# JialeTao/MRFA

Hardware: AMD Instinct MI355X
Metric: frames/sec (256x256 source+driving pair) fwd+bwd (higher is better)
Workload: dtype f32; 1 GPU; vox1.yaml MTIA (TokenPose_B) prior + DenseMotion + RaftFlow refinement, 256x256, bs=8/GPU, fwd+bwd+clip+Adam, train-mode BN, surrogate L1 loss; global_batch=8, parallelism=dp1, prior=mtia, background_predictor=False, sync_bn=False, launch=hipGraph, optimizer=FlatAdam (K20), mfma=bf16x6

## Files before the change

mrfa_amd/build.py:

```python
import glob
import os
import subprocess
import sys

HERE = os.path.dirname(os.path.abspath(__file__))
ROOT = os.path.dirname(HERE)
CSRC = os.path.join(HERE, "csrc")
LIBDIR = os.path.join(HERE, "_lib")
LIB = os.path.join(LIBDIR, "libmrfa_hip.so")
SOURCES = ["error.cpp", "conv_plan.hip", "conv_mfma.hip", "conv_split.hip", "conv_halo.hip", "conv_small.hip", "conv_lean.hip", "wgrad_mfma.hip", "wgrad_split.hip", "wgrad_halo.hip", "wgrad_small.hip", "wgrad_lean.hip", "conv_fewout.hip", "conv_fewout3.hip", "layout.hip", "pack_multi.hip", "norm.hip", "sample.hip", "elementwise.hip", "optim.hip", "tokenpose.hip", "attention_mfma.hip", "losses.hip", "prior.hip", "pose.hip", "metrics.hip", "frames.hip"]
FLAGS = ["--offload-arch=gfx950", "-O3", "-std=c++17", "-fPIC", "-I" + os.path.join(ROOT, "include"), "-I" + CSRC,
         "-Wno-unused-result"]
CSRC_DATA = os.path.join(HERE, "csrc_data")
DATA_LIB = os.path.join(LIBDIR, "libmrfa_data_hip.so")
DATA_FLAGS = FLAGS + ["-I" + CSRC_DATA, "-ffp-contract=off", "-fhip-fp32-correctly-rounded-divide-sqrt"]


def _stale(out, deps):
    if not os.path.exists(out):
        return True
    t = os.path.getmtime(out)
    return any(os.path.getmtime(d) > t for d in deps)


def data_sources() -> list:
    return ["error.cpp"] + sorted(os.path.basename(p) for p in glob.glob(os.path.join(CSRC_DATA, "*.hip")))


def build(force: bool = False, verbose: bool = True) -> str:
    os.makedirs(LIBDIR, exist_ok=True)
    hipcc = os.environ.get("HIPCC", "/opt/rocm/bin/hipcc")
    headers = [os.path.join(ROOT, "include", "mrfa_hip.h")] + sorted(glob.glob(os.path.join(CSRC, "*.h")))
    data_headers = headers + [os.path.join(ROOT, "include", h) for h in ("mrfa_data_hip.h", "mrfa_resize_hip.h")] \
        + sorted(glob.glob(os.path.join(CSRC_DATA, "*.h")))
    units = [(CSRC, src, "", FLAGS, headers) for src in SOURCES] + [(CSRC_DATA, src, "data_", DATA_FLAGS, data_headers) for src in data_sources()]
    objs = {LIB: [], DATA_LIB: []}
    procs = []
    for srcdir, src, prefix, flags, deps in units:
        sp = os.path.join(srcdir, src)
        if not os.path.exists(sp):
            raise FileNotFoundError(sp)
        obj = os.path.join(LIBDIR, prefix + os.path.splitext(src)[0] + ".o")
        objs[DATA_LIB if prefix else LIB].append(obj)
        if force or _stale(obj, [sp] + deps):
            cmd = [hipcc] + flags + (["-x", "hip"] if src.endswith(".cpp") else []) + ["-c", sp, "-o", obj]
            if verbose:
                print("[mrfa_amd.build]", " ".join(cmd), flush=True)
            procs.append((src, subprocess.Popen(cmd)))
    for src, pr in procs:
        if pr.wait() != 0:
            raise RuntimeError(f"hipcc failed on {src}")
    for out, os_ in objs.items():
        if force or _stale(out, os_):
            cmd = [hipcc, "--offload-arch=gfx950", "-shared", "-fPIC", "-o", out] + os_
            if verbose:
                print("[mrfa_amd.build]", " ".join(cmd), flush=True)
            subprocess.check_call(cmd)
    return LIB


if __name__ == "__main__":
    build(force="--force" in sys.argv)
    print(LIB)
    print(DATA_LIB)
```

mrfa_amd/csrc/common.h:

```cpp
#pragma once
#include <hip/hip_runtime.h>
#include <stdio.h>
#include <string.h>
#include "mrfa_hip.h"

typedef float f32x16 __attribute__((ext_vector_type(16)));
typedef float f32x4 __attribute__((ext_vector_type(4)));

void mrfa_set_error(const char* fmt, ...);

struct MrfaTuning {
    int conv_small;
    int conv_halo, conv_halo_min_tiles, conv_halo_pr, conv_halo_phase, conv_halo_bn256, conv_halo_bn192, conv_halo_bn64_fill;
    int conv_lean, conv_lean_min_wgs, conv_lean_geo, gemm_lean;
    int wgrad_halo, wgrad_halo_min_wgs, wgrad_halo_target_wgs, wgrad_halo_phase, wgrad_lean;
    int conv_fewout3, attention_mfma;
};
extern MrfaTuning g_tune;

struct HaloGeo { int PR, BN; bool phase; };

enum class ConvFamily { lean, gemm_lean, small, halo, halo_dgrad, rows_split, rows_f32, refused };
struct ConvPlan {
    ConvFamily family;
    char error[256];
    long long M;
    int KT;
    int lean_geo, gemm_cfg, small_tm, small_tn;
    HaloGeo halo;
    int BM, BN, splitk;
    bool w8;
    bool fused;
    bool fin_in_launch;
    bool reads_w;
    int last_config;
    bool groups_ok, bst_ok, stride2_ok, mask_ok, phase_dgrad_ok;
};
ConvPlan plan_conv(const mrfa_conv_params& p);

enum class WgradFamily { lean, small, halo, tiled, refused };
struct WgradPlan {
    WgradFamily family;
    char error[192];
    long long M;
    bool lean, small;
    bool groups_ok, stride2_ok;
};
WgradPlan plan_wgrad(const mrfa_wgrad_params& p);

int mrfa_conv_split_launch(hipStream_t st, const mrfa_conv_params& p, int KT, long long M, int splitk, int BN);
bool mrfa_conv_halo_eligible(const mrfa_conv_params& p, HaloGeo* geo);
int mrfa_conv_halo_launch(hipStream_t st, const mrfa_conv_params& p, const HaloGeo& geo);
int mrfa_wgrad_split_launch(hipStream_t st, const mrfa_wgrad_params& p, dim3 grid, long long M, long long kps, int tiles_n, int nsplit, int inner,
                            int total_splits, int taps, long long partial_stride, int BM, int BN);

bool mrfa_wgrad_halo_eligible(const mrfa_wgrad_params& p);
int mrfa_wgrad_halo_launch(hipStream_t st, const mrfa_wgrad_params& p);

bool mrfa_fewout3_wgrad(hipStream_t st, const float* x, int ldx, int N, int H, int W, int Cin, const float* dy, int lddy, int Cout, int R, int pad,
                        float* dw, float* dbias, int* rc);

int mrfa_conv_lean_pick(const mrfa_conv_params& p);
int mrfa_conv_lean_launch(hipStream_t st, const mrfa_conv_params& p, int geo);
int mrfa_gemm_lean_pick(const mrfa_conv_params& p, long long M);
int mrfa_gemm_lean_launch(hipStream_t st, const mrfa_conv_params& p, long long M, int cfg);

bool mrfa_conv_small_eligible(const mrfa_conv_params& p, long long M);
int mrfa_conv_small_launch(hipStream_t st, const mrfa_conv_params& p, long long M, int tm, int tn);

bool mrfa_attention_mfma_ok(int d, int n, const void* qkv, int ld, const void* out, int ldo, const void* dout, int lddo, const void* dqkv, int lddq);
int mrfa_attention_fwd_mfma(hipStream_t st, const float* qkv, int ld, int B, int n, int heads, int d, float scale, float* out, int ldo, float* lse);
int mrfa_attention_bwd_mfma(hipStream_t st, const float* qkv, int ld, const float* out, int ldo, const float* dout, int lddo, const float* lse,
                            float* delta, int B, int n, int heads, int d, float scale, float* dqkv, int lddq);

bool mrfa_wgrad_lean_eligible(const mrfa_wgrad_params& p);
int mrfa_wgrad_lean_multi(hipStream_t st, const mrfa_wgrad_params* ps, int n, unsigned char* taken);

bool mrfa_wgrad_small_eligible(const mrfa_wgrad_params& p, long long M);
int mrfa_wgrad_small_launch(hipStream_t st, const mrfa_wgrad_params& p, long long M);

#define MRFA_CHECK_ARG(cond, ...)                      \
    do {                                               \
        if (!(cond)) {                                 \
            mrfa_set_error(__VA_ARGS__);               \
            return 1;                                  \
        }                                              \
    } while (0)

#define MRFA_CHECK_LAUNCH(name)                                                   \
    do {                                                                          \
        hipError_t e_ = hipGetLastError();                                        \
        if (e_ != hipSuccess) {                                                   \
            mrfa_set_error("%s: launch failed: %s", name, hipGetErrorString(e_)); \
            return 2;                                                             \
        }                                                                         \
    } while (0)

static inline bool aligned16(const void* p) { return (reinterpret_cast<uintptr_t>(p) & 15u) == 0; }
static inline int cdiv(long long a, long long b) { return (int)((a + b - 1) / b); }

static inline int stream_grid(long long work_items, int block) {
    long long g = (work_items + block - 1) / block;
    if (g < 1) g = 1;
    if (g > 256 * 16) g = 256 * 16;
    return (int)g;
}

__device__ __forceinline__ int xcd_tile_index() {
    const int per_xcd = (int)gridDim.x >> 3;
    return (int)(blockIdx.x & 7) * per_xcd + (int)(blockIdx.x >> 3);
}

__device__ __forceinline__ void chain_prio() {
    __builtin_amdgcn_s_setprio(3);
}

__device__ __forceinline__ int stat_group(const mrfa_conv_params& p, long long row, long long M) {
    return p.groups > 1 ? (int)(row / (M / p.groups)) : 0;
}
__device__ __forceinline__ double* stat_slot(const mrfa_conv_params& p, int group, unsigned slot) {
    return p.stats + ((size_t)group * MRFA_STATS_SLOTS + slot % MRFA_STATS_SLOTS) * 2 * p.Cout;
}
static inline long long group_rows(const mrfa_conv_params& p, long long M) {
    if (p.groups <= 1) return M;
    return (p.N % p.groups) == 0 ? M / p.groups : 0;
}

__device__ __forceinline__ bool splitk_last_arriver(unsigned* ticket, unsigned nsplit) {
    __shared__ unsigned s_sk_ticket;
    asm volatile("s_waitcnt vmcnt(0)" ::: "memory");
    __syncthreads();
    if (threadIdx.x == 0) s_sk_ticket = __hip_atomic_fetch_add(ticket, 1u, __ATOMIC_RELAXED, __HIP_MEMORY_SCOPE_AGENT);
    __syncthreads();
    return s_sk_ticket == nsplit - 1;
}

__device__ __forceinline__ bool fin_last_arriver(unsigned* counter, unsigned participants, int idx) {
    __shared__ unsigned s_fin_ticket;
    asm volatile("s_waitcnt vmcnt(0)" ::: "memory");
    __syncthreads();
    if (threadIdx.x == 0) {
        if (idx < 0) {
            s_fin_ticket = __hip_atomic_fetch_add(counter, 1u, __ATOMIC_RELAXED, __HIP_MEMORY_SCOPE_AGENT) == participants - 1;
        } else {
            const unsigned nsh = participants < 8u ? participants : 8u, sh = (unsigned)idx % nsh;
            const unsigned mine = participants / nsh + (sh < participants % nsh ? 1u : 0u);
            unsigned last = 0;
            if (__hip_atomic_fetch_add(counter + 1 + sh, 1u, __ATOMIC_RELAXED, __HIP_MEMORY_SCOPE_AGENT) == mine - 1)
                last = __hip_atomic_fetch_add(counter, 1u, __ATOMIC_RELAXED, __HIP_MEMORY_SCOPE_AGENT) == nsh - 1;
            s_fin_ticket = last;
        }
    }
    __syncthreads();
    return s_fin_ticket != 0;
}

__device__ __forceinline__ double fin_slot_sum(const double* first, size_t stride) {
    double v[MRFA_STATS_SLOTS];
#pragma unroll
    for (int s = 0; s < MRFA_STATS_SLOTS; ++s) v[s] = __hip_atomic_load(first + (size_t)s * stride, __ATOMIC_RELAXED, __HIP_MEMORY_SCOPE_AGENT);
    double t = 0.0;
#pragma unroll
    for (int s = 0; s < MRFA_STATS_SLOTS; ++s) t += v[s];
    return t;
}

__device__ __forceinline__ void fused_bn_finalize(const mrfa_conv_params& p, unsigned participants, int idx = -1, double* scratch = nullptr, int scratch_n = 0) {
    if (!fin_last_arriver(p.fin_counter, participants, idx)) return;
    const double cnt = (double)p.fin_count;
    const int G = p.groups > 1 ? p.groups : 1;
    const int C2 = 2 * p.Cout;
    const bool par = scratch != nullptr && scratch_n >= G * C2;
    if (par) {
        for (int o = threadIdx.x; o < G * C2; o += blockDim.x) scratch[o] = fin_slot_sum(p.stats + (size_t)(o / C2) * MRFA_STATS_SLOTS * C2 + o % C2, (size_t)C2);
        __syncthreads();
    }
    for (int c = threadIdx.x; c < p.Cout; c += blockDim.x) {
        float rm = p.fin_rmean ? p.fin_rmean[c] : 0.f, rv = p.fin_rmean ? p.fin_rvar[c] : 0.f;
        for (int g = 0; g < G; ++g) {
            const double* sg = p.stats + (size_t)g * MRFA_STATS_SLOTS * C2;
            const double t1 = par ? scratch[g * C2 + c] : fin_slot_sum(sg + c, (size_t)C2);
            const double t2 = par ? scratch[g * C2 + p.Cout + c] : fin_slot_sum(sg + p.Cout + c, (size_t)C2);
            const double m = t1 / cnt;
            double var = t2 / cnt - m * m;
            if (var < 0.0) var = 0.0;
            const float mean = (float)m, invstd = (float)(1.0 / sqrt(var + (double)p.fin_eps));
            const double unb = p.fin_count > 1 ? var * cnt / (cnt - 1.0) : var;
            rm = (1.f - p.fin_momentum) * rm + p.fin_momentum * mean;
            rv = (1.f - p.fin_momentum) * rv + p.fin_momentum * (float)unb;
            const float sc = p.fin_gamma[c] * invstd;
            const int gc = g * p.Cout + c;
            p.fin_scale[gc] = sc;
            p.fin_shift[gc] = p.fin_beta[c] - mean * sc;
            if (p.fin_mean) p.fin_mean[gc] = mean;
            if (p.fin_invstd) p.fin_invstd[gc] = invstd;
        }
        if (p.fin_rmean) { p.fin_rmean[c] = rm; p.fin_rvar[c] = rv; }
    }
}

__device__ __forceinline__ float wave_sum(float v) {
#pragma unroll
    for (int o = 32; o > 0; o >>= 1) v += __shfl_xor(v, o, 64);
    return v;
}
```

mrfa_amd/csrc/conv_plan.hip:

```cpp
#include "common.h"
#include <stdarg.h>

MrfaTuning g_tune = {
     1,
     1,  128,  0,  1,  1,
     1,  1,
     1,  128,  -1,
     1,
     1,  192,  256,  1,
     1,
     1,  1,
};

enum TuneKind { T_ON, T_INT, T_NONNEG, T_NONNEG_ON, T_LEVEL, T_POS };
static const struct { const char* key; int* field; TuneKind kind; } TUNING_KEYS[] = {
    {"conv_small", &g_tune.conv_small, T_ON},
    {"conv_halo", &g_tune.conv_halo, T_ON},
    {"conv_halo_min_tiles", &g_tune.conv_halo_min_tiles, T_INT},
    {"conv_halo_pr", &g_tune.conv_halo_pr, T_INT},
    {"conv_halo_phase", &g_tune.conv_halo_phase, T_ON},
    {"conv_halo_bn256", &g_tune.conv_halo_bn256, T_ON},
    {"conv_halo_bn192", &g_tune.conv_halo_bn192, T_ON},
    {"conv_halo_bn64_fill", &g_tune.conv_halo_bn64_fill, T_ON},
    {"conv_lean", &g_tune.conv_lean, T_ON},
    {"conv_lean_min_wgs", &g_tune.conv_lean_min_wgs, T_NONNEG},
    {"conv_lean_geo", &g_tune.conv_lean_geo, T_INT},
    {"gemm_lean", &g_tune.gemm_lean, T_LEVEL},
    {"wgrad_halo", &g_tune.wgrad_halo, T_ON},
    {"wgrad_halo_min_wgs", &g_tune.wgrad_halo_min_wgs, T_NONNEG},
    {"wgrad_halo_target_wgs", &g_tune.wgrad_halo_target_wgs, T_POS},
    {"wgrad_halo_phase", &g_tune.wgrad_halo_phase, T_NONNEG_ON},
    {"wgrad_lean", &g_tune.wgrad_lean, T_ON},
    {"conv_fewout3", &g_tune.conv_fewout3, T_ON},
    {"attention_mfma", &g_tune.attention_mfma, T_ON},
};

extern "C" int mrfa_set_tuning(const char* key, int value) {
    if (!key) return -1;
    for (const auto& k : TUNING_KEYS) {
        if (strcmp(key, k.key)) continue;
        const int prev = *k.field;
        switch (k.kind) {
            case T_ON: *k.field = value != 0; break;
            case T_INT: *k.field = value; break;
            case T_NONNEG: if (value >= 0) *k.field = value; break;
            case T_NONNEG_ON: if (value >= 0) *k.field = value != 0; break;
            case T_LEVEL: if (value >= 0) *k.field = value > 2 ? 2 : value; break;
            case T_POS: if (value > 0) *k.field = value; break;
        }
        return prev;
    }
    return -1;
}

namespace {
constexpr int BK = 32;

template <typename Plan>
Plan& refuse(Plan& c, const char* fmt, ...) {
    va_list ap;
    va_start(ap, fmt);
    vsnprintf(c.error, sizeof(c.error), fmt, ap);
    va_end(ap);
    c.family = decltype(c.family)::refused;
    return c;
}

void plan_rows(ConvPlan& c, const mrfa_conv_params& p, int mode) {
    const bool flat = p.kflat > 0;
    const long long M = c.M;
    const int KT = c.KT;
    const int nb = p.nbatch > 1 ? p.nbatch : 1;
    int BN = 128;
    {
        const int cands[4] = {128, 96, 64, 32};
        const double pen[4] = {1.0, 1.08, 1.16, 1.3};
        double best = 1e18;
        for (int i = 0; i < 4; ++i) {
            if (cands[i] == 96 && flat) continue;
            const double cost = (double)cdiv(p.Cout, cands[i]) * cands[i] * pen[i];
            if (cost < best) { best = cost; BN = cands[i]; }
        }
    }
    if (mode >= 1 && !flat && p.Cout >= 32) BN = p.Cout <= 64 ? 64 : 128;
    auto ntiles = [&](int bm, int bn) { return ((M + bm - 1) / bm) * cdiv(p.Cout, bn) * nb; };
    int BM = 128;
    if (BN == 96 && ntiles(128, 96) < 384) BN = 128;
    if (BN == 128) { if (M <= 32) BM = 32; else if (M <= 64) BM = 64; }
    else if (BN == 64 && M <= 64) BM = 64;
    int splitk = 1;
    const bool auto_split = (p.splitk == 0);
    if (p.splitk > 1) splitk = p.splitk;
    {
        const bool short_k_big_m = KT < 32 && M > 4096;
        const bool grouped_stats = p.groups > 1 && p.stats && !(p.sk_ticket && !p.accumulate);
        const int max_split = (auto_split && !short_k_big_m && !grouped_stats) ? (KT / 2 > 0 ? KT / 2 : 1) : 1;
        long long t = ntiles(BM, BN);
        if (t < 384 && !(short_k_big_m && t >= 128)) {
            const bool half_target = auto_split && p.sk_ticket && !p.accumulate && KT >= 72 && KT <= 320 && BM == 128 && t >= 8 && t <= 16;
            int want = (int)(((half_target ? 256 : 512) + t - 1) / t);
            if (auto_split) splitk = want <= max_split ? want : max_split;
            const int min_bm = (BN == 128) ? 32 : (BN == 64 ? 64 : 128);
            while (!half_target && ntiles(BM, BN) * splitk < 384 && BM > min_bm) {
                BM >>= 1;
                if (auto_split) {
                    t = ntiles(BM, BN);
                    want = (int)((512 + t - 1) / t);
                    splitk = want <= max_split ? want : max_split;
                }
            }
            if (splitk < 1) splitk = 1;
        }
    }
    bool w8 = false;
    if (p.tile) {
        BM = p.tile >> 16; BN = p.tile & 0x7fff; w8 = (p.tile & 0x8000) != 0;
        if (p.splitk >= 1) splitk = p.splitk;
    } else if (BM == 128 && BN == 128 && !flat) {
        w8 = true;
    }
    const bool split_operand = mode >= 1 && BM == 128 && (BN == 128 || BN == 64) && !flat;
    c.family = split_operand ? ConvFamily::rows_split : ConvFamily::rows_f32;
    c.BM = BM;
    c.BN = BN;
    c.w8 = w8;
    c.splitk = splitk;
    c.fused = splitk > 1 && p.sk_ticket && !p.accumulate;
    c.fin_in_launch = p.fin_scale && nb == 1 && (splitk == 1 || c.fused);
    c.reads_w = !(split_operand && mode != 3 && p.w_split);
    c.last_config = (BM << 16) | (BN << 4) | ((flat ? 1 : 0) << 1) | (splitk > 1 ? 1 : 0) | (split_operand ? 4 : 0);
}
}

ConvPlan plan_conv(const mrfa_conv_params& p) {
    ConvPlan c = {};
    const int mode = mrfa_get_mfma_mode();
    const bool flat = p.kflat > 0;
    c.M = (long long)p.N * p.Hout * p.Wout;
    c.KT = ((flat ? p.kflat : p.R * p.S * p.Cin) + BK - 1) / BK;
    c.splitk = 1;
    c.reads_w = true;
    c.fin_in_launch = p.fin_scale != nullptr;

    c.lean_geo = flat ? -1 : mrfa_conv_lean_pick(p);
    c.gemm_cfg = (flat || c.lean_geo >= 0) ? -1 : mrfa_gemm_lean_pick(p, c.M);
    const bool lean = c.lean_geo >= 0, gemm = c.gemm_cfg >= 0;
    const bool small = !lean && !gemm && g_tune.conv_small && mrfa_conv_small_eligible(p, c.M);
    const bool halo = !flat && mrfa_conv_halo_eligible(p, &c.halo);

    const long long rows = group_rows(p, c.M);
    c.groups_ok = p.groups <= 1 || !(p.stats || p.fin_scale || p.bst_x || p.in_scale) ||
                  (p.nbatch <= 1 && p.splitk <= 1 && rows > 0 &&
                   (lean || gemm || (!p.in_scale && ((rows % 128) == 0 || small || (p.stride <= 1 && halo)))));
    c.bst_ok = p.stats && !p.fin_scale && p.stride >= 0 && !flat && (lean || gemm || small);
    c.stride2_ok = p.stride == 2 && p.Hout == (p.Hin + 2 * p.pad - p.R) / 2 + 1 && p.Wout == (p.Win + 2 * p.pad - p.S) / 2 + 1 &&
                   (flat ? (!p.ups && p.nbatch <= 1 && p.splitk <= 1 && p.ktab) : small);
    c.mask_ok = halo;
    c.phase_dgrad_ok = p.ups == 2 && halo;

    if (!(p.x && p.w)) return refuse(c, "conv2d: null pointer");
    if (!(p.N > 0 && p.Cin > 0 && p.Cout > 0 && p.Hout > 0 && p.Wout > 0)) return refuse(c, "conv2d: bad sizes");
    if (!(p.R >= 1 && p.S >= 1 && p.R <= 15 && p.S <= 15)) return refuse(c, "conv2d: kernel size %dx%d unsupported", p.R, p.S);
    if (!((p.w_ld % 4) == 0 && aligned16(p.w))) return refuse(c, "conv2d: packed weight must be 16-B aligned, w_ld %% 4 == 0");
    if (!flat && (p.Cin % 32) != 0) return refuse(c, "conv2d: chunked mode needs Cin %% 32 == 0 (got %d); use flat mode", p.Cin);
    if (!flat && !((p.ldx % 4) == 0 && aligned16(p.x))) return refuse(c, "conv2d: chunked mode needs 16-B aligned x and ldx %% 4 == 0");
    if (!flat && p.in_scale && !(aligned16(p.in_scale) && aligned16(p.in_shift))) return refuse(c, "conv2d: in_scale/in_shift alignment");
    if (flat && !(p.ktab != nullptr && aligned16(p.ktab))) return refuse(c, "conv2d: flat mode needs a 16-B aligned ktab");
    if (lean) {
        c.family = ConvFamily::lean;
        c.reads_w = false;
        c.last_config = (32 << 16) | (32 << 4) | 4 | (1 << 27);
        return c;
    }
    if (gemm) {
        c.family = ConvFamily::gemm_lean;
        c.reads_w = false;
        c.last_config = (64 << 16) | (64 << 4) | 4 | (1 << 26);
        return c;
    }
    if (small) {
        c.family = ConvFamily::small;
        const int ncols = (p.Cout + 15) / 16 * 16;
        auto waves = [&](int wm, int wn) { return ((c.M + wm - 1) / wm) * ((ncols + wn - 1) / wn); };
        int tm = 2, tn = 2;
        if (waves(32, 32) < 2048) { tm = 1; tn = 2; }
        if (tm == 1 && waves(16, 32) < 2048) { tn = 1; }
        if (ncols % 32 != 0 && tn == 2 && ncols < 32) tn = 1;
        if (p.groups > 1 && tm == 2 && (rows % 128) != 0) tm = 1;
        c.small_tm = tm;
        c.small_tn = tn;
        c.last_config = (16 << 16) | (16 << 4) | 8;
        return c;
    }
    if (p.stride < 0 || p.stride > 2 || (p.stride == 2 && !(flat && !p.ups && p.nbatch <= 1)))
        return refuse(c, "conv2d: stride = %d is only implemented by the one-wave-per-tile kernel and by flat-K launches: ask mrfa_conv2d_stride_supported() first", p.stride);
    if (p.mask && !halo) return refuse(c, "conv2d: `mask` is only honoured by the patch-tiled kernel: ask mrfa_conv2d_mask_supported() first");
    if (p.ups == 2 && !halo)
        return refuse(c, "conv2d: ups = 2 (phase data gradient of a fused-upsample layer) is only implemented for the shapes mrfa_conv2d_phase_dgrad_supported() reports");
    if (halo) {
        c.family = p.ups == 2 ? ConvFamily::halo_dgrad : ConvFamily::halo;
        c.reads_w = false;
        c.last_config = (128 << 16) | ((p.Cout <= 64 ? 64 : 128) << 4) | 4 | (1 << 28);
        return c;
    }
    plan_rows(c, p, mode);
    return c;
}

WgradPlan plan_wgrad(const mrfa_wgrad_params& p) {
    WgradPlan c = {};
    const bool flat = p.kflat > 0;
    c.M = (long long)p.N * p.Hout * p.Wout;
    c.lean = mrfa_wgrad_lean_eligible(p);
    c.small = g_tune.conv_small && mrfa_wgrad_small_eligible(p, c.M);
    c.groups_ok = p.groups <= 1 || !p.in_scale || c.lean;
    c.stride2_ok = p.stride == 2 && p.Hout == (p.Hin + 2 * p.pad - p.R) / 2 + 1 && p.Wout == (p.Win + 2 * p.pad - p.S) / 2 + 1 && c.small;
    if (!(p.x && p.dy && p.dw)) return refuse(c, "wgrad: null pointer");
    if (!flat && !((p.ldx % 4) == 0 && aligned16(p.x))) return refuse(c, "wgrad: x must be a 16-B aligned view with ld %% 4 == 0");
    if (flat && !p.ktab) return refuse(c, "wgrad: flat mode needs ktab");
    if (!(c.M < (1ll << 31) - 64)) return refuse(c, "wgrad: too many pixels");
    if (p.in_scale && c.lean) { c.family = WgradFamily::lean; return c; }
    if (!c.groups_ok) return refuse(c, "wgrad: groups = %d with a prologue is only implemented where mrfa_conv2d_wgrad_groups_supported() says so", p.groups);
    if (c.small) { c.family = WgradFamily::small; return c; }
    if (p.stride > 1) return refuse(c, "wgrad: stride = %d is only implemented by the small-problem kernel: ask mrfa_conv2d_wgrad_stride_supported() first", p.stride);
    c.family = !flat && mrfa_wgrad_halo_eligible(p) ? WgradFamily::halo : WgradFamily::tiled;
    return c;
}

extern "C" int mrfa_conv2d_split_k(const mrfa_conv_params* p) {
    if (!p) return 1;
    if (p->splitk > 1) return p->splitk;
    const ConvPlan c = plan_conv(*p);
    return c.family == ConvFamily::refused ? 1 : c.splitk;
}

extern "C" int mrfa_conv2d_reads_fp32_weights(const mrfa_conv_params* p) {
    if (!p) return 1;
    const ConvPlan c = plan_conv(*p);
    return c.family == ConvFamily::refused || c.reads_w ? 1 : 0;
}

extern "C" int mrfa_conv2d_groups_supported(const mrfa_conv_params* p) { return p && plan_conv(*p).groups_ok ? 1 : 0; }
extern "C" int mrfa_conv2d_bwdstats_supported(const mrfa_conv_params* p) { return p && plan_conv(*p).bst_ok ? 1 : 0; }
extern "C" int mrfa_conv2d_stride_supported(const mrfa_conv_params* p) { return p && plan_conv(*p).stride2_ok ? 1 : 0; }
extern "C" int mrfa_conv2d_mask_supported(const mrfa_conv_params* p) { return p && plan_conv(*p).mask_ok ? 1 : 0; }
extern "C" int mrfa_conv2d_phase_dgrad_supported(const mrfa_conv_params* p) { return p && plan_conv(*p).phase_dgrad_ok ? 1 : 0; }

extern "C" int mrfa_conv2d_wgrad_stride_supported(const mrfa_wgrad_params* p) { return p && plan_wgrad(*p).stride2_ok ? 1 : 0; }
extern "C" int mrfa_conv2d_wgrad_groups_supported(const mrfa_wgrad_params* p) { return p && plan_wgrad(*p).groups_ok ? 1 : 0; }
extern "C" int mrfa_conv2d_wgrad_lean_supported(const mrfa_wgrad_params* p) { return p && plan_wgrad(*p).lean ? 1 : 0; }
```

mrfa_amd/csrc/wgrad_mfma.hip:

```cpp
#include "common.h"
#include <stdlib.h>
#include <algorithm>

namespace {

constexpr int WBK = 32;
constexpr int KG = WBK / 4;

template <int BM, int BN, int WAVES_M, int WAVES_N, bool FLAT, bool ROWAL>
__global__ __launch_bounds__(WAVES_M * WAVES_N * 64) void wgrad_mfma_kernel(const mrfa_wgrad_params p, const long long M, const long long k_per_split,
                                                        const int tiles_n, const int nsplit, const int dy_scalar,
                                                        const int inner, const int total_splits, const int taps,
                                                        const long long partial_stride) {
    constexpr int WTM = BM / WAVES_M, WTN = BN / WAVES_N;
    constexpr int TM = WTM / 32, TN = WTN / 32;
    constexpr int NT = WAVES_M * WAVES_N * 64;
    static_assert((NT == 256 || NT == 512) && TM >= 1 && TN >= 1, "tile");
    constexpr int SA = BM / 4 + 4, SB = BN / 4 + 4;
    constexpr int PLA = 4 * SA, PLB = 4 * SB;
    constexpr int IA = (BM / 4) * KG, IB = (BN / 4) * KG;
    __shared__ f32x4 smem[2 * KG * (PLA + PLB)];

    const int tid = threadIdx.x, lane = tid & 63, wave = tid >> 6;
    const int wm = wave / WAVES_N, wn = wave % WAVES_N;
// ... 156 lines not shown
                }
            }
            ra[rr] = v;
        }
        int n_img = b_n, oy = b_oy, ox = b_ox;
#pragma unroll
        for (int rr = 0; rr < 4; ++rr) {
            const int pp = k0 + 4 * b_kg + rr;
            f32x4 v = {0.f, 0.f, 0.f, 0.f};
            if (pp < ke && b_any) {
                if constexpr (!FLAT) {
                    const int iy = oy + r - p.pad, ix = ox + s - p.pad;
                    if ((unsigned)iy < (unsigned)Hv && (unsigned)ix < (unsigned)Wv) {
                        const size_t pix = (size_t)n_img * p.Hin * p.Win + (size_t)(iy >> p.ups) * p.Win + (ix >> p.ups);
                        v = *reinterpret_cast<const f32x4*>(x + pix * p.ldx + ci0 + b_col);
                        if (p.in_scale) {
                            v = v * sc + sh;
                            if (p.in_relu) { v.x = fmaxf(v.x, 0.f); v.y = fmaxf(v.y, 0.f); v.z = fmaxf(v.z, 0.f); v.w = fmaxf(v.w, 0.f); }
                        }
#pragma unroll
                        for (int q = 0; q < 4; ++q) if (!cmask[q]) v[q] = 0.f;
                    }
                } else {
#pragma unroll
                    for (int q = 0; q < 4; ++q) {
                        const int iy = oy + fdy[q], ix = ox + fdx[q];
                        if (cmask[q] && (unsigned)iy < (unsigned)Hv && (unsigned)ix < (unsigned)Wv) {
                            const size_t pix = (size_t)n_img * p.Hin * p.Win + (size_t)(iy >> p.ups) * p.Win + (ix >> p.ups);
                            float t = x[pix * p.ldx + fci[q]];
                            if (p.in_scale) { t = t * sc[q] + sh[q]; if (p.in_relu) t = fmaxf(t, 0.f); }
                            v[q] = t;
                        }
                    }
                }
            }
            rb[rr] = v;
            if (++ox == p.Wout) { ox = 0; if (++oy == p.Hout) { oy = 0; ++n_img; } }
        }
        b_ox += WBK;
        while (b_ox >= p.Wout) {
            b_ox -= p.Wout;
            if (++b_oy == p.Hout) { b_oy = 0; ++b_n; }
        }
    };
    auto store_tiles = [&](int buf) {
        f32x4* As = smem + buf * KG * (PLA + PLB);
        f32x4* Bs = As + KG * PLA;
        if (a_item) {
#pragma unroll
            for (int e = 0; e < 4; ++e) As[a_kg * PLA + e * SA + a_cg] = f32x4{ra[0][e], ra[1][e], ra[2][e], ra[3][e]};
            if (do_bias) bias_acc += ra[0] + ra[1] + ra[2] + ra[3];
        }
        if (b_item) {
#pragma unroll
            for (int e = 0; e < 4; ++e) Bs[b_kg * PLB + e * SB + b_cg] = f32x4{rb[0][e], rb[1][e], rb[2][e], rb[3][e]};
        }
    };

    f32x16 acc[TM][TN];
#pragma unroll
    for (int i = 0; i < TM; ++i)
#pragma unroll
        for (int j = 0; j < TN; ++j)
#pragma unroll
            for (int q = 0; q < 16; ++q) acc[i][j][q] = 0.f;

    if (kb < ke) {
        load_tiles(kb);
        store_tiles(0);
    }
    __syncthreads();
    const int fi = lane & 31, fh = lane >> 5;
    const int a_lane = (fi & 3) * SA + (fi >> 2) + ((wm * WTM) >> 2);
    const int b_lane = (fi & 3) * SB + (fi >> 2) + ((wn * WTN) >> 2);
    int cur = 0;
    for (int k0 = kb; k0 < ke; k0 += WBK) {
        const bool more = (k0 + WBK) < ke;
        if (more) load_tiles(k0 + WBK);
        const f32x4* As = smem + cur * KG * (PLA + PLB) + a_lane;
        const f32x4* Bs = smem + cur * KG * (PLA + PLB) + KG * PLA + b_lane;
#pragma unroll
        for (int q = 0; q < KG / 2; ++q) {
            f32x4 a[TM], b[TN];
#pragma unroll
            for (int i = 0; i < TM; ++i) a[i] = As[(2 * q + fh) * PLA + i * 8];
#pragma unroll
            for (int j = 0; j < TN; ++j) b[j] = Bs[(2 * q + fh) * PLB + j * 8];
#pragma unroll
            for (int e = 0; e < 4; ++e)
#pragma unroll
                for (int i = 0; i < TM; ++i)
#pragma unroll
                    for (int j = 0; j < TN; ++j)
                        acc[i][j] = __builtin_amdgcn_mfma_f32_32x32x2f32(a[i][e], b[j][e], acc[i][j], 0, 0, 0);
        }
        if (more) store_tiles(cur ^ 1);
        __syncthreads();
        cur ^= 1;
    }

#pragma unroll
    for (int j = 0; j < TN; ++j) {
        const int nn = ci0 + wn * WTN + j * 32 + (lane & 31);
        if (nn >= NTOT) continue;
        const int otap = FLAT ? nn / p.Cin : tap;
        const int ci = FLAT ? nn - otap * p.Cin : nn;
#pragma unroll
        for (int i = 0; i < TM; ++i) {
#pragma unroll
            for (int q = 0; q < 16; ++q) {
                const int co = co0 + wm * WTM + i * 32 + (q & 3) + 8 * (q >> 2) + 4 * fh;
                if (co < p.Cout) {
                    const size_t idx = ((size_t)otap * p.Cout + co) * p.Cin + ci;
                    if (partial_stride) p.ws[(size_t)split * partial_stride + idx] = acc[i][j][q] * p.alpha;
                    else atomicAdd(dw + idx, acc[i][j][q] * p.alpha);
                }
            }
        }
    }
    if (p.dbias != nullptr && tap == 0 && tile_n == 0) {
        float* red = reinterpret_cast<float*>(smem);
        __syncthreads();
        if (a_item) {
#pragma unroll
            for (int q = 0; q < 4; ++q) red[a_kg * BM + a_col + q] = bias_acc[q];
        }
        __syncthreads();
        if (tid < BM && co0 + tid < p.Cout) {
            float sacc = 0.f;
#pragma unroll
            for (int g = 0; g < KG; ++g) sacc += red[g * BM + tid];
            atomicAdd(p.dbias + co0 + tid, sacc);
        }
    }
}


__global__ void wgrad_reduce_kernel(const float* __restrict__ ws, float* __restrict__ dw, long long n, int nsplit) {
    const int groups = (nsplit + 15) / 16;
    const long long total = n * groups;
    for (long long t = blockIdx.x * (long long)blockDim.x + threadIdx.x; t < total; t += (long long)gridDim.x * blockDim.x) {
        const int g = (int)(t / n);
        const long long i = t - (long long)g * n;
        const int k0 = g * 16, k1 = min(nsplit, k0 + 16);
        float s = 0.f;
#pragma unroll 16
        for (int k = k0; k < k1; ++k) s += ws[(size_t)k * n + i];
        atomicAdd(dw + i, s);
    }
}

}

extern "C" int mrfa_conv2d_wgrad_nhwc(void* stream, const mrfa_wgrad_params* pp) {
    const mrfa_wgrad_params& p = *pp;
    hipStream_t st = (hipStream_t)stream;
    const WgradPlan c = plan_wgrad(p);
    const long long M = c.M;
    switch (c.family) {
        case WgradFamily::refused: mrfa_set_error("%s", c.error); return 1;
        case WgradFamily::lean: { unsigned char taken = 0; return mrfa_wgrad_lean_multi(st, &p, 1, &taken); }
        case WgradFamily::small: return mrfa_wgrad_small_launch(st, p, M);
        case WgradFamily::halo: return mrfa_wgrad_halo_launch(st, p);
        case WgradFamily::tiled: break;
    }
    const int dy_scalar = ((p.ldy % 4) == 0 && aligned16(p.dy) && (p.dy_bs % 4) == 0) ? 0 : 1;
    const bool flat = p.kflat > 0;
    const int nb = p.nbatch > 1 ? p.nbatch : 1;
    int taps = flat ? 1 : p.R * p.S;
    const int NTOT = flat ? p.kflat : p.Cin;
    auto pick = [](int n) {
        const int cands[4] = {128, 96, 64, 32};
        const double pen[4] = {1.0, 1.12, 1.35, 1.8};
        int best_t = 128;
        double best = 1e18;
        for (int i = 0; i < 4; ++i) {
            const double cost = (double)cdiv(n, cands[i]) * cands[i] * pen[i];
            if (cost < best) { best = cost; best_t = cands[i]; }
        }
        return best_t;
    };
    int BM = pick(p.Cout), BN = pick(NTOT);
    if (BM < 128 && BN < 128) {
        if (BM == 64 && BN == 64) {}
        else if (BM <= BN) BN = 128;
        else BM = 128;
    }
    if (flat && (BM == 96 || BN == 96)) { BM = BM == 96 ? 128 : BM; BN = BN == 96 ? 128 : BN; }
    const bool split_mode = mrfa_get_mfma_mode() >= 1 && !flat && (p.Wout % 8) == 0 && (M % WBK) == 0 && !dy_scalar && p.Cout >= 32 && NTOT >= 32;
    if (split_mode) { BM = p.Cout <= 64 ? 64 : 128; BN = NTOT <= 64 ? 64 : 128; if (BM == 64 && BN == 64) BN = 128; }
    int tiles_m = cdiv(p.Cout, BM), tiles_n = cdiv(NTOT, BN);
    int taps_arg = taps;
    constexpr bool cflat_on = true;
    if (cflat_on && split_mode && taps > 1 && (p.Cin % 4) == 0) {
        const double per_tap = (double)taps * tiles_n * BN * (BN == 64 ? 1.4 : 1.0), flat_w = (double)cdiv(taps * p.Cin, 128) * 128;
        if (flat_w <= 0.85 * per_tap) {
            BN = 128;
            tiles_n = cdiv(taps * p.Cin, 128);
            taps = 1;
            taps_arg = -1;
        }
    }
    const long long base = (long long)tiles_m * tiles_n * taps * nb;
    int nsplit = p.ksplit;
    if (nsplit <= 0) {
        const long long max_split = std::max<long long>(1, M / (8 * WBK));
        double best = 1e30;
        nsplit = 1;
        const long long inner_ = (long long)tiles_m * tiles_n * taps;
        for (long long ns = 1; ns <= std::min<long long>(max_split, 1024); ++ns) {
            const long long S = ns * nb;
            const long long ktiles = ((M + ns - 1) / ns + WBK - 1) / WBK;
            double rounds;
            if (S >= 8) rounds = (double)(((S + 7) / 8 * inner_ + 63) / 64);
            else rounds = (double)((S * inner_ + 511) / 512);
            const double cost = rounds * (double)(ktiles + 6);
            if (cost < best * 0.999) { best = cost; nsplit = (int)ns; }
        }
    }
    long long kps = (M + nsplit - 1) / nsplit;
    kps = (kps + WBK - 1) / WBK * WBK;
    nsplit = (int)((M + kps - 1) / kps);
    const int inner = tiles_m * tiles_n * taps;
    const int total_splits = nsplit * nb;
    const long long wn = (long long)(flat ? 1 : taps) * 0 + (long long)p.R * p.S * p.Cout * p.Cin;
    const long long partial_stride = (nb == 1 && nsplit >= 24 && p.ws && wn * nsplit * 4 <= p.ws_bytes) ? wn : 0;
    dim3 grid((unsigned)(cdiv(total_splits, 8) * 8 * inner));
    const bool rowal = (p.Wout % WBK) == 0;
#define WLAUNCH(bm, bn, wm, wn, fl, ra)                                                                                     \
    hipLaunchKernelGGL((wgrad_mfma_kernel<bm, bn, wm, wn, fl, ra>), grid, dim3((wm) * (wn) * 64), 0, st, p, M, kps, tiles_n, nsplit, dy_scalar, \
                       inner, total_splits, taps, partial_stride)
#define WCFG(bm, bn, wm, wn)                                              \
    if (BM == bm && BN == bn) {                                           \
        if (flat && rowal) WLAUNCH(bm, bn, wm, wn, true, true);           \
        else if (flat) WLAUNCH(bm, bn, wm, wn, true, false);              \
        else if (rowal) WLAUNCH(bm, bn, wm, wn, false, true);             \
        else WLAUNCH(bm, bn, wm, wn, false, false);                       \
    }
    if (split_mode) {
        const int rc = mrfa_wgrad_split_launch(st, p, grid, M, kps, tiles_n, nsplit, inner, total_splits, taps_arg, partial_stride, BM, BN);
        if (rc) return rc;
    }
    else if (BM == 128 && BN == 128 && !flat && rowal && !p.tile8_off) { WLAUNCH(128, 128, 2, 4, false, true); }
    else WCFG(128, 128, 2, 2)
    else WCFG(128, 64, 2, 2)
    else WCFG(64, 128, 2, 2)
    else WCFG(64, 64, 2, 2)
    else WCFG(32, 128, 1, 4)
    else WCFG(128, 32, 4, 1)
    else WCFG(128, 96, 4, 1)
    else WCFG(96, 128, 1, 4)
    else { mrfa_set_error("wgrad: no tile config"); return 1; }
#undef WCFG
#undef WLAUNCH
    MRFA_CHECK_LAUNCH("mrfa_conv2d_wgrad_nhwc");
    if (partial_stride) {
        hipLaunchKernelGGL(wgrad_reduce_kernel, dim3(stream_grid(wn * ((nsplit + 15) / 16), 256)), dim3(256), 0, st, p.ws, p.dw, wn, nsplit);
        MRFA_CHECK_LAUNCH("wgrad_reduce");
    }
    return 0;
}
```

Measured before the change: 102.5 pairs/s.

## Add specialized MFMA weight-gradient kernel for few-input-channel flat convolutions

Adds a dedicated wgrad kernel for convolutions with at most 4 input channels (e.g. the first 7x7 conv on RGB input) in flattened-K mode. It streams dy and a rolling ring of padded input rows through LDS, double-buffered, and builds the tap-expanded B operand on the fly from LDS instead of going through the generic tiled im2col path. It then reduces across waves and writes either split partials or atomics, with a fused bias reduction. The goal is to stop the generic tiled wgrad from wasting MFMA work and memory traffic on tiny Cin, at the cost of a new complex code path and a planner branch.

```diff
diff --git a/mrfa_amd/build.py b/mrfa_amd/build.py
--- a/mrfa_amd/build.py
+++ b/mrfa_amd/build.py
@@ -8,7 +8,7 @@
 CSRC = os.path.join(HERE, "csrc")
 LIBDIR = os.path.join(HERE, "_lib")
 LIB = os.path.join(LIBDIR, "libmrfa_hip.so")
-SOURCES = ["error.cpp", "conv_plan.hip", "conv_mfma.hip", "conv_split.hip", "conv_halo.hip", "conv_small.hip", "conv_lean.hip", "wgrad_mfma.hip", "wgrad_split.hip", "wgrad_halo.hip", "wgrad_small.hip", "wgrad_lean.hip", "conv_fewout.hip", "conv_fewout3.hip", "layout.hip", "pack_multi.hip", "norm.hip", "sample.hip", "elementwise.hip", "optim.hip", "tokenpose.hip", "attention_mfma.hip", "losses.hip", "prior.hip", "pose.hip", "metrics.hip", "frames.hip"]
+SOURCES = ["error.cpp", "conv_plan.hip", "conv_mfma.hip", "conv_split.hip", "conv_halo.hip", "conv_small.hip", "conv_lean.hip", "wgrad_mfma.hip", "wgrad_split.hip", "wgrad_halo.hip", "wgrad_small.hip", "wgrad_lean.hip", "wgrad_fewin.hip", "conv_fewout.hip", "conv_fewout3.hip", "layout.hip", "pack_multi.hip", "norm.hip", "sample.hip", "elementwise.hip", "optim.hip", "tokenpose.hip", "attention_mfma.hip", "losses.hip", "prior.hip", "pose.hip", "metrics.hip", "frames.hip"]
 FLAGS = ["--offload-arch=gfx950", "-O3", "-std=c++17", "-fPIC", "-I" + os.path.join(ROOT, "include"), "-I" + CSRC,
          "-Wno-unused-result"]
 CSRC_DATA = os.path.join(HERE, "csrc_data")
diff --git a/mrfa_amd/csrc/common.h b/mrfa_amd/csrc/common.h
--- a/mrfa_amd/csrc/common.h
+++ b/mrfa_amd/csrc/common.h
@@ -15,6 +15,7 @@
     int conv_lean, conv_lean_min_wgs, conv_lean_geo, gemm_lean;
     int wgrad_halo, wgrad_halo_min_wgs, wgrad_halo_target_wgs, wgrad_halo_phase, wgrad_lean;
     int conv_fewout3, attention_mfma;
+    int conv_fewin;
 };
 extern MrfaTuning g_tune;
 
@@ -38,7 +39,7 @@
 };
 ConvPlan plan_conv(const mrfa_conv_params& p);
 
-enum class WgradFamily { lean, small, halo, tiled, refused };
+enum class WgradFamily { lean, small, halo, fewin, tiled, refused };
 struct WgradPlan {
     WgradFamily family;
     char error[192];
@@ -56,6 +57,10 @@
 
 bool mrfa_wgrad_halo_eligible(const mrfa_wgrad_params& p);
 int mrfa_wgrad_halo_launch(hipStream_t st, const mrfa_wgrad_params& p);
+
+bool mrfa_wgrad_fewin_eligible(const mrfa_wgrad_params& p);
+int mrfa_wgrad_fewin_launch(hipStream_t st, const mrfa_wgrad_params& p);
+int mrfa_wgrad_reduce_launch(hipStream_t st, const float* ws, float* dw, long long n, int nsplit);
 
 bool mrfa_fewout3_wgrad(hipStream_t st, const float* x, int ldx, int N, int H, int W, int Cin, const float* dy, int lddy, int Cout, int R, int pad,
                         float* dw, float* dbias, int* rc);
diff --git a/mrfa_amd/csrc/conv_plan.hip b/mrfa_amd/csrc/conv_plan.hip
--- a/mrfa_amd/csrc/conv_plan.hip
+++ b/mrfa_amd/csrc/conv_plan.hip
@@ -10,6 +10,7 @@
      1,  192,  256,  1,
      1,
      1,  1,
+     1,
 };
 
 enum TuneKind { T_ON, T_INT, T_NONNEG, T_NONNEG_ON, T_LEVEL, T_POS };
@@ -33,6 +34,7 @@
     {"wgrad_lean", &g_tune.wgrad_lean, T_ON},
     {"conv_fewout3", &g_tune.conv_fewout3, T_ON},
     {"attention_mfma", &g_tune.attention_mfma, T_ON},
+    {"conv_fewin", &g_tune.conv_fewin, T_ON},
 };
 
 extern "C" int mrfa_set_tuning(const char* key, int value) {
@@ -223,6 +225,7 @@
     if (!c.groups_ok) return refuse(c, "wgrad: groups = %d with a prologue is only implemented where mrfa_conv2d_wgrad_groups_supported() says so", p.groups);
     if (c.small) { c.family = WgradFamily::small; return c; }
     if (p.stride > 1) return refuse(c, "wgrad: stride = %d is only implemented by the small-problem kernel: ask mrfa_conv2d_wgrad_stride_supported() first", p.stride);
+    if (flat && mrfa_wgrad_fewin_eligible(p)) { c.family = WgradFamily::fewin; return c; }
     c.family = !flat && mrfa_wgrad_halo_eligible(p) ? WgradFamily::halo : WgradFamily::tiled;
     return c;
 }
diff --git a/mrfa_amd/csrc/wgrad_fewin.hip b/mrfa_amd/csrc/wgrad_fewin.hip
--- /dev/null
+++ b/mrfa_amd/csrc/wgrad_fewin.hip
@@ -0,0 +1,315 @@
+#include <stdlib.h>
+#include "mfma_bf16.h"
+
+namespace {
+
+constexpr int NT = 256;
+constexpr int SR = 2;
+constexpr int PXS = 32 * SR;
+constexpr int RING = 16;
+constexpr int HPW = 32 + 7 - 1;
+constexpr int ROWF = HPW * 4;
+constexpr int DYBLK = PXS * 64;
+constexpr int MB = 2;
+
+__device__ __forceinline__ bf16x8 as_frag(const u32x4& v) {
+    bf16x8 r;
+    __builtin_memcpy(&r, &v, 16);
+    return r;
+}
+
+template <int NBW, int WN, int NP>
+__global__ __launch_bounds__(NT) __attribute__((amdgpu_waves_per_eu(2, 2))) void wgrad_fewin_kernel(const mrfa_wgrad_params p, const int tiles_co, const int HS,
+                                                                                                const int segs_y, const int tiles_x, const int total,
+                                                                                                const long long partial_stride) {
+    constexpr int WK = 4 / WN;
+    constexpr int NPC = NP == 6 ? 3 : (NP == 3 ? 2 : 1);
+    constexpr int DYBUF = NPC * MB * DYBLK;
+    constexpr int XBYTES = RING * ROWF * 4;
+    constexpr int STAGE = 2 * DYBUF + XBYTES;
+    constexpr int WTILE = MB * NBW * 16 * 64;
+    constexpr int RED = (WK - 1) * WN * WTILE * 4;
+    constexpr int NDY = 2 * MB;
+    static_assert(WN * WK == 4 && MB * NBW <= 6, "four waves, <= 96 accumulator registers");
+    __shared__ __attribute__((aligned(16))) unsigned char smem[STAGE > RED ? STAGE : RED];
+    unsigned char* const smD = smem;
+    f32x4* const smX = reinterpret_cast<f32x4*>(smem + 2 * DYBUF);
+    const float* const smXf = reinterpret_cast<const float*>(smem + 2 * DYBUF);
+
+    const int tid = threadIdx.x, lane = tid & 63, wave = tid >> 6;
+    const int wn = wave % WN, wk = wave / WN;
+    const int lin = blockIdx.x;
+    if (lin >= total) return;
+    const int tile_co = lin % tiles_co;
+    const int seg = lin / tiles_co;
+    const int ys = seg % segs_y;
+    const int xt = (seg / segs_y) % tiles_x;
+    const int n_img = seg / (segs_y * tiles_x);
+    const int co0 = tile_co * 32 * MB;
+    const int y0 = ys * HS, y1 = min(p.Hout, y0 + HS), x0 = xt * 32;
+    const int Ntot = p.kflat;
+
+    const float* __restrict__ x = p.x;
+    const float* __restrict__ dy = p.dy;
+
+    const int d_col = tid >> 3, d_quad = tid & 7;
+    const bool d_colok = x0 + d_col < p.Wout;
+    const int d_gbase = (n_img * p.Hout * p.Wout + min(x0 + d_col, p.Wout - 1)) * p.ldy + co0 + d_quad * 4;
+    const int d_lbase = d_col * 64 + d_quad * 8;
+    bool d_blkok[MB];
+#pragma unroll
+    for (int b = 0; b < MB; ++b) d_blkok[b] = co0 + b * 32 < p.Cout;
+    const bool x_act = tid < SR * HPW;
+    const int x_r = x_act ? tid / HPW : 0, x_hp = x_act ? tid - x_r * HPW : 0;
+    const int x_ix = x0 - p.pad + x_hp;
+    const bool x_colok = x_act && (unsigned)x_ix < (unsigned)p.Win;
+    const int x_gbase = (n_img * p.Hin * p.Win + (x_colok ? x_ix : 0)) * 4;
+
+    f32x4 rd[NDY], rx, bsum[MB];
+#pragma unroll
+    for (int b = 0; b < MB; ++b) bsum[b] = f32x4{0.f, 0.f, 0.f, 0.f};
+
+    auto load_x = [&](int row0) {
+        const int yc = min(max(row0 + x_r, 0), p.Hin - 1);
+        rx = *reinterpret_cast<const f32x4*>(x + (size_t)x_gbase + (size_t)yc * p.Win * 4);
+    };
+    auto store_x = [&](int row0) {
+        const int iy = row0 + x_r;
+        const f32x4 z = {0.f, 0.f, 0.f, 0.f};
+        const f32x4 v = (x_colok && (unsigned)iy < (unsigned)p.Hin) ? rx : z;
+        if (x_act) smX[((iy + 2 * RING) & (RING - 1)) * HPW + x_hp] = v;
+    };
+    auto load_d = [&](int oa) {
+#pragma unroll
+        for (int j = 0; j < NDY; ++j) {
+            const int yc = min(oa + (j & 1), p.Hout - 1);
+            rd[j] = *reinterpret_cast<const f32x4*>(dy + (size_t)d_gbase + (d_blkok[j >> 1] ? (j >> 1) * 32 : 0) + (size_t)yc * p.Wout * p.ldy);
+        }
+    };
+    auto store_d = [&](int oa, int buf) {
+        unsigned char* dst = smD + buf * DYBUF + d_lbase;
+#pragma unroll
+        for (int j = 0; j < NDY; ++j) {
+            const bool ok = d_colok && d_blkok[j >> 1] && (oa + (j & 1)) < y1;
+            const f32x4 z = {0.f, 0.f, 0.f, 0.f};
+            const f32x4 v = ok ? rd[j] : z;
+            bsum[j >> 1] += v;
+            u32x2 p1, p2, p3;
+            bf16_pieces<NP>(v, p1, p2, p3);
+            unsigned char* d = dst + (j >> 1) * DYBLK + (j & 1) * 32 * 64;
+            *reinterpret_cast<u32x2*>(d) = p1;
+            if constexpr (NPC >= 2) *reinterpret_cast<u32x2*>(d + MB * DYBLK) = p2;
+            if constexpr (NPC == 3) *reinterpret_cast<u32x2*>(d + 2 * MB * DYBLK) = p3;
+        }
+    };
+
+    int b_off[NBW], b_r[NBW];
+    bool b_ok[NBW];
+#pragma unroll
+    for (int j = 0; j < NBW; ++j) {
+        const int n = 32 * (wn + j * WN) + (lane & 31);
+        b_ok[j] = n < Ntot;
+        const int nn = b_ok[j] ? n : 0;
+        const int tap = nn / p.Cin, ci = nn - tap * p.Cin;
+        const int r = tap / p.S, s = tap - r * p.S;
+        b_r[j] = r - p.pad + 2 * RING;
+        b_off[j] = (s + 8 * (lane >> 5)) * 4 + ci;
+    }
+    const int nblocks = (Ntot + 31) >> 5;
+
+    f32x16 acc[MB][NBW];
+#pragma unroll
+    for (int m = 0; m < MB; ++m)
+#pragma unroll
+        for (int j = 0; j < NBW; ++j)
+#pragma unroll
+            for (int r = 0; r < 16; ++r) acc[m][j][r] = 0.f;
+
+    const int l16 = lane & 15, grp = lane >> 4;
+    const int frag_off = (8 * (grp >> 1) + (l16 >> 2)) * 64 + (grp & 1) * 32 + (l16 & 3) * 8;
+
+    auto compute = [&](int oa, int buf) {
+        const unsigned char* D = smD + buf * DYBUF + frag_off;
+#pragma unroll
+        for (int kq = 0; kq < WN; ++kq) {
+            const int kk = wk * WN + kq;
+            bf16x8 a[NPC][MB];
+#pragma unroll
+            for (int pc = 0; pc < NPC; ++pc)
+#pragma unroll
+                for (int m = 0; m < MB; ++m) a[pc][m] = tr_frag(D + (pc * MB + m) * DYBLK + kk * 16 * 64);
+#pragma unroll
+            for (int j = 0; j < NBW; ++j) {
+                if (wn + j * WN >= nblocks) continue;
+                const float* xp = smXf + ((oa + (kk >> 1) + b_r[j]) & (RING - 1)) * ROWF + b_off[j] + (kk & 1) * 64;
+                float xv[8];
+#pragma unroll
+                for (int i = 0; i < 8; ++i) xv[i] = b_ok[j] ? xp[4 * i] : 0.f;
+                u32x4 q1, q2, q3;
+                bf16_pieces<NP>(xv, q1, q2, q3);
+                bf16x8 b[NPC];
+                b[0] = as_frag(q1);
+                if constexpr (NPC >= 2) b[1] = as_frag(q2);
+                if constexpr (NPC == 3) b[2] = as_frag(q3);
+#pragma unroll
+                for (int t = 6 - NP; t < 6; ++t)
+#pragma unroll
+                    for (int m = 0; m < MB; ++m) acc[m][j] = __builtin_amdgcn_mfma_f32_32x32x16_bf16(a[PA[t]][m], b[PB[t]], acc[m][j], 0, 0, 0);
+            }
+        }
+    };
+
+    for (int r0 = y0 - p.pad; r0 < y0 - p.pad + p.R + 1; r0 += SR) {
+        load_x(r0);
+        store_x(r0);
+    }
+    load_d(y0);
+    store_d(y0, 0);
+    load_x(y0 + SR - p.pad + p.R - 1);
+    load_d(y0 + SR);
+    __syncthreads();
+    int buf = 0;
+    for (int oa = y0; oa < y1; oa += SR) {
+        store_x(oa + SR - p.pad + p.R - 1);
+        store_d(oa + SR, buf ^ 1);
+        load_x(oa + 2 * SR - p.pad + p.R - 1);
+        load_d(oa + 2 * SR);
+        compute(oa, buf);
+        __syncthreads();
+        buf ^= 1;
+    }
+
+    if constexpr (WK > 1) {
+        float* red = reinterpret_cast<float*>(smem);
+        if (wk > 0) {
+            float* dst = red + ((wk - 1) * WN + wn) * WTILE + lane;
+#pragma unroll
+            for (int m = 0; m < MB; ++m)
+#pragma unroll
+                for (int j = 0; j < NBW; ++j)
+#pragma unroll
+                    for (int r = 0; r < 16; ++r) dst[((m * NBW + j) * 16 + r) * 64] = acc[m][j][r];
+        }
+        __syncthreads();
+        if (wk == 0) {
+#pragma unroll
+            for (int g = 0; g < WK - 1; ++g) {
+                const float* src = red + (g * WN + wn) * WTILE + lane;
+#pragma unroll
+                for (int m = 0; m < MB; ++m)
+#pragma unroll
+                    for (int j = 0; j < NBW; ++j)
+#pragma unroll
+                        for (int r = 0; r < 16; ++r) acc[m][j][r] += src[((m * NBW + j) * 16 + r) * 64];
+            }
+        }
+    }
+
+    if (wk == 0) {
+        float* __restrict__ out = partial_stride ? p.ws + (size_t)seg * partial_stride : p.dw;
+        const int half = lane >> 5;
+#pragma unroll
+        for (int j = 0; j < NBW; ++j) {
+            const int n = 32 * (wn + j * WN) + (lane & 31);
+            if (n >= Ntot) continue;
+            const int tap = n / p.Cin, ci = n - tap * p.Cin;
+#pragma unroll
+            for (int m = 0; m < MB; ++m) {
+#pragma unroll
+                for (int r = 0; r < 16; ++r) {
+                    const int co = co0 + m * 32 + (r & 3) + 8 * (r >> 2) + 4 * half;
+                    if (co < p.Cout) {
+                        const size_t idx = ((size_t)tap * p.Cout + co) * p.Cin + ci;
+                        if (partial_stride) out[idx] = acc[m][j][r] * p.alpha;
+                        else atomicAdd(out + idx, acc[m][j][r] * p.alpha);
+                    }
+                }
+            }
+        }
+    }
+    if (p.dbias != nullptr) {
+        float* red = reinterpret_cast<float*>(smem);
+        __syncthreads();
+        if (tid < 32 * MB) red[tid] = 0.f;
+        __syncthreads();
+#pragma unroll
+        for (int b = 0; b < MB; ++b) {
+            f32x4 v = bsum[b];
+#pragma unroll
+            for (int e = 0; e < 4; ++e) {
+                float s = v[e];
+                s += __shfl_xor(s, 8, 64);
+                s += __shfl_xor(s, 16, 64);
+                s += __shfl_xor(s, 32, 64);
+                v[e] = s;
+            }
+            if ((lane >> 3) == 0) {
+#pragma unroll
+                for (int e = 0; e < 4; ++e) atomicAdd(red + b * 32 + d_quad * 4 + e, v[e]);
+            }
+        }
+        __syncthreads();
+        if (tid < 32 * MB && co0 + tid < p.Cout) atomicAdd(p.dbias + co0 + tid, red[tid]);
+    }
+}
+
+struct FewinGeo { int NBW, WN, tiles_co, tiles_x, HS, segs_y; long long total; };
+
+FewinGeo fewin_geo(const mrfa_wgrad_params& p) {
+    FewinGeo g = {};
+    const int nb = cdiv(p.kflat, 32);
+    if (nb == 1) { g.WN = 1; g.NBW = 1; }
+    else if (nb <= 4) { g.WN = 4; g.NBW = 1; }
+    else if (nb <= 6) { g.WN = 2; g.NBW = 3; }
+    else { g.WN = 4; g.NBW = 2; }
+    g.tiles_co = cdiv(p.Cout, 32 * MB);
+    g.tiles_x = cdiv(p.Wout, 32);
+    const long long cols = (long long)p.N * g.tiles_x * g.tiles_co;
+    const int slots = 512;
+    g.HS = p.Hout;
+    double best = (double)((cols + slots - 1) / slots) * (p.Hout + 8);
+    for (int hs = 8; hs < p.Hout; hs *= 2) {
+        const long long tot = cols * cdiv(p.Hout, hs);
+        const double cost = (double)((tot + slots - 1) / slots) * (hs + 8);
+        if (cost < best) { best = cost; g.HS = hs; }
+    }
+    g.segs_y = cdiv(p.Hout, g.HS);
+    g.total = cols * g.segs_y;
+    return g;
+}
+
+template <int NBW, int WN>
+void fewin_launch_np(hipStream_t st, const mrfa_wgrad_params& p, const FewinGeo& g, long long partial_stride) {
+    const int mode = mrfa_get_mfma_mode();
+    const dim3 grid((unsigned)g.total), block(NT);
+    if (mode == 3) hipLaunchKernelGGL((wgrad_fewin_kernel<NBW, WN, 1>), grid, block, 0, st, p, g.tiles_co, g.HS, g.segs_y, g.tiles_x, (int)g.total, partial_stride);
+    else if (mode == 2) hipLaunchKernelGGL((wgrad_fewin_kernel<NBW, WN, 3>), grid, block, 0, st, p, g.tiles_co, g.HS, g.segs_y, g.tiles_x, (int)g.total, partial_stride);
+    else hipLaunchKernelGGL((wgrad_fewin_kernel<NBW, WN, 6>), grid, block, 0, st, p, g.tiles_co, g.HS, g.segs_y, g.tiles_x, (int)g.total, partial_stride);
+}
+
+}
+
+bool mrfa_wgrad_fewin_eligible(const mrfa_wgrad_params& p) {
+    const int mode = mrfa_get_mfma_mode();
+    if (!g_tune.conv_fewin || (mode != 1 && mode != 2 && mode != 3)) return false;
+    if (p.Cin < 1 || p.Cin > 4 || p.ldx != 4 || !aligned16(p.x) || p.kflat != p.R * p.S * p.Cin) return false;
+    if (p.R < 1 || p.S < 1 || p.R > 7 || p.S > 7 || p.pad < 0 || p.pad > 7 || p.stride > 1 || p.ups || p.in_scale || p.nbatch > 1 || p.ksplit > 0) return false;
+    if (p.Cout < 32 || (p.Cout % 32) != 0 || (p.ldy % 4) != 0 || !aligned16(p.dy)) return false;
+    if (p.Hout != p.Hin + 2 * p.pad - p.R + 1 || p.Wout != p.Win + 2 * p.pad - p.S + 1 || p.Hout < 1 || p.Wout < 1) return false;
+    if ((long long)p.N * p.Hin * p.Win * 4 >= (1ll << 31) || (long long)p.N * p.Hout * p.Wout * p.ldy >= (1ll << 31)) return false;
+    return fewin_geo(p).total < (1ll << 31);
+}
+
+int mrfa_wgrad_fewin_launch(hipStream_t st, const mrfa_wgrad_params& p) {
+    const FewinGeo g = fewin_geo(p);
+    const long long wn = (long long)p.R * p.S * p.Cout * p.Cin;
+    const long long nsplit = g.total / g.tiles_co;
+    const long long partial_stride = (p.ws && wn * nsplit * 4 <= p.ws_bytes) ? wn : 0;
+    if (g.NBW == 1 && g.WN == 1) fewin_launch_np<1, 1>(st, p, g, partial_stride);
+    else if (g.NBW == 1) fewin_launch_np<1, 4>(st, p, g, partial_stride);
+    else if (g.NBW == 3) fewin_launch_np<3, 2>(st, p, g, partial_stride);
+    else fewin_launch_np<2, 4>(st, p, g, partial_stride);
+    MRFA_CHECK_LAUNCH("mrfa_conv2d_wgrad_nhwc(fewin)");
+    if (partial_stride) return mrfa_wgrad_reduce_launch(st, p.ws, p.dw, wn, (int)nsplit);
+    return 0;
+}
diff --git a/mrfa_amd/csrc/wgrad_mfma.hip b/mrfa_amd/csrc/wgrad_mfma.hip
--- a/mrfa_amd/csrc/wgrad_mfma.hip
+++ b/mrfa_amd/csrc/wgrad_mfma.hip
@@ -332,6 +332,12 @@
 
 }
 
+int mrfa_wgrad_reduce_launch(hipStream_t st, const float* ws, float* dw, long long n, int nsplit) {
+    hipLaunchKernelGGL(wgrad_reduce_kernel, dim3(stream_grid(n * ((nsplit + 15) / 16), 256)), dim3(256), 0, st, ws, dw, n, nsplit);
+    MRFA_CHECK_LAUNCH("wgrad_reduce");
+    return 0;
+}
+
 extern "C" int mrfa_conv2d_wgrad_nhwc(void* stream, const mrfa_wgrad_params* pp) {
     const mrfa_wgrad_params& p = *pp;
     hipStream_t st = (hipStream_t)stream;
@@ -342,6 +348,7 @@
         case WgradFamily::lean: { unsigned char taken = 0; return mrfa_wgrad_lean_multi(st, &p, 1, &taken); }
         case WgradFamily::small: return mrfa_wgrad_small_launch(st, p, M);
         case WgradFamily::halo: return mrfa_wgrad_halo_launch(st, p);
+        case WgradFamily::fewin: return mrfa_wgrad_fewin_launch(st, p);
         case WgradFamily::tiled: break;
     }
     const int dy_scalar = ((p.ldy % 4) == 0 && aligned16(p.dy) && (p.dy_bs % 4) == 0) ? 0 : 1;
@@ -435,8 +442,7 @@
 #undef WLAUNCH
     MRFA_CHECK_LAUNCH("mrfa_conv2d_wgrad_nhwc");
     if (partial_stride) {
-        hipLaunchKernelGGL(wgrad_reduce_kernel, dim3(stream_grid(wn * ((nsplit + 15) / 16), 256)), dim3(256), 0, st, p.ws, p.dw, wn, nsplit);
-        MRFA_CHECK_LAUNCH("wgrad_reduce");
+        return mrfa_wgrad_reduce_launch(st, p.ws, p.dw, wn, nsplit);
     }
     return 0;
 }
```

New measurement: 103.9 pairs/s, median of 3. About the same (+1.4%).
